# arnavdantuluri/StableTriton

Hardware: AMD Instinct MI355X
Metric: denoise it/s, SDXL UNet 1024x1024 50-step, bs=1 per GPU (higher is better)
Workload: dtype bf16; 1 GPU; SDXL-base UNet, latent 128x128 (1024x1024 px), bs=1/GPU, 50-step Euler-discrete loop, hipGraph mode=step, no CFG; parallelism=prompt-parallel x1, weights=synthetic seed 0, weight_broadcasts=0

## Files before the change

### stabletriton_amd/csrc/dispatch.h

```cpp
#pragma once
#include "gemm_reg.h"
#include "gemm_dma.h"
#include "gemm8p.h"
#ifdef ST_DEV_CONFIGS
#include "../../tools/dev_kernels/gemm4w.h"
void gemm4w_bf16(const GemmArgs& a, hipStream_t st);
void gemm4w_f16(const GemmArgs& a, hipStream_t st);
void gemm4w_fp8(const GemmArgs& a, hipStream_t st);
template <typename T> static inline void gemm4w_call(const GemmArgs& a, hipStream_t st) {
    if constexpr (std::is_same<T, bf16>::value) gemm4w_bf16(a, st);
    else if constexpr (std::is_same<T, f16>::value) gemm4w_f16(a, st);
    else gemm4w_fp8(a, st);
}
#endif

static inline bool colstats_ok(const GemmArgs& a, int bm, bool lnf) {
    const bool ok = a.col_stats && !lnf && (a.N & 3) == 0 && a.rows_per_batch > 0 && a.rows_per_batch % bm == 0 &&
                    cdiv(a.M, bm) <= a.col_tiles_cap;
    if (a.col_rows_out) *a.col_rows_out = ok ? bm : 0;
    return ok;
}

template <typename T, int BM, int BN, int WGM, int WGN, int STAGES, int U, bool CONV, bool GEGLU, bool LNF, bool XA = false>
static void launch_dma_one(const GemmArgs& a, hipStream_t st, int tiles_n) {
    const size_t lds = (size_t)STAGES * U * (BM + BN) * 128 + (size_t)BM * 8 + 1024;
    const int sk = a.splitk > 1 ? a.splitk : 1;
    auto kfn = gemm_dma_kernel<T, BM, BN, WGM, WGN, STAGES, U, CONV, GEGLU, LNF, XA>;
    const bool emit_cols = colstats_ok(a, BM, LNF);
    static unsigned long long lds_ok = 0;
    ensure_dynamic_lds(kfn, lds, &lds_ok);
    GemmArgs b = a;
    {
        static const int force_pm = dev_env_int("ST_GEMM_PANELS", 0);
        const int tiles_m = cdiv(a.M, BM);
        const double abytes = CONV ? (double)a.M * a.Cin * (a.ups ? 0.25 : 1.0) * a.stride * a.stride : (double)a.M * a.K;
        const double wbytes = (double)(GEGLU ? 2 : 1) * a.N * a.K;
        int best_p = 1;
        double best = 1e300;
        for (int pm = 1; pm <= 8; pm *= 2) {
            if (pm > tiles_m) break;
            const double c = abytes * (8.0 / pm) + wbytes * pm;
            if (c < best) { best = c; best_p = pm; }
        }
        if (force_pm > 0) best_p = force_pm > tiles_m ? tiles_m : force_pm;
        b.panel_h = cdiv(tiles_m, best_p);
    }
    const int main_blocks = cdiv(a.M, BM) * tiles_n * sk;
    b.splitk = sk;
    fill_tile_map(b, cdiv(a.M, BM), tiles_n, a.K / ((128 / (int)sizeof(T)) * U));
    static const bool no_helpers = dev_env_int("ST_NO_HELPER_BLOCKS", 0) != 0;
    b.helper_blocks = (b.next_w && main_blocks <= 208 && !no_helpers) ? (256 - main_blocks > 96 ? 96 : 256 - main_blocks) : 0;
    if (!emit_cols) b.col_stats = nullptr;
    fill_next_per(b, main_blocks + b.helper_blocks);
    hipLaunchKernelGGL(kfn, dim3(main_blocks + b.helper_blocks), dim3(WGM * WGN * 64), lds, st, b);
}

template <typename T, int BM, int BN, int WGM, int WGN, int STAGES, int U, bool CONV>
static void launch_dma(const GemmArgs& a, hipStream_t st) {
    if constexpr (!CONV) {
        const bool geglu = a.epi & ST_EPI_GEGLU;
        constexpr bool PAIRS = (BN % 32 == 0);
        if (a.ln_c) {
            if constexpr (PAIRS) {
                if (geglu) { launch_dma_one<T, BM, BN, WGM, WGN, STAGES, U, false, true, true>(a, st, cdiv(a.N, BN / 2)); return; }
            }
            launch_dma_one<T, BM, BN, WGM, WGN, STAGES, U, false, false, true>(a, st, cdiv(a.N, BN));
            return;
        }
        if constexpr (PAIRS) {
            if (geglu) { launch_dma_one<T, BM, BN, WGM, WGN, STAGES, U, false, true, false>(a, st, cdiv(a.N, BN / 2)); return; }
        }
    }
    launch_dma_one<T, BM, BN, WGM, WGN, STAGES, U, CONV, false, false>(a, st, cdiv(a.N, BN));
}

enum { CFG_64x64_S4 = 0, CFG_64x64_S8 = 1, CFG_64x64_S4_U2 = 2, CFG_128x64_S4 = 3, CFG_128x64_S3_U2 = 4,
       CFG_128x128_S3 = 5, CFG_64x64_S3 = 6, CFG_64x64_W8 = 7, CFG_128x64_W8 = 8, CFG_128x128_W8 = 9,
       CFG_64x128_W8 = 10, CFG_64x128_W8_S6 = 11, CFG_128x64_W8_S6 = 12, CFG_128x128_W8_S4 = 13, CFG_64x64_W8_S8 = 14, CFG_64x128_W8_U2 = 15, CFG_128x64_W8_U2 = 16, CFG_64x64_W8_U2 = 17, CFG_256x256_W8 = 18, CFG_256x128_W8 = 19, CFG_128x128_W8_S2 = 20, CFG_128x64_W8_S3 = 21, CFG_64x128_W8_S3 = 22, CFG_128x320_W8 = 23, CFG_128x256_W8 = 24, CFG_64x320_W8 = 25, CFG_64x80_W4 = 26, CFG_128x80_W8 = 27, CFG_128x160_W8 = 28, CFG_128x128_N4_S2 = 29, CFG_128x64_N4_S3 = 30, CFG_64x128_N4_S3 = 31, CFG_256x160_W8_S2 = 32, CFG_COUNT, CFG_256x256_8P = 100, CFG_256x160_8P = 101, CFG_256x256_4W = 102 };

static inline int cfg_bn(int cfg) {
    switch (cfg) {
        case CFG_64x64_S4: case CFG_64x64_S8: case CFG_64x64_S4_U2: case CFG_128x64_S4: case CFG_128x64_S3_U2: case CFG_64x64_S3:
        case CFG_64x64_W8: case CFG_128x64_W8: case CFG_128x64_W8_S6: case CFG_64x64_W8_S8: case CFG_128x64_W8_U2:
        case CFG_64x64_W8_U2: case CFG_128x64_W8_S3: case CFG_128x64_N4_S3: return 64;
        case CFG_256x256_W8: case CFG_128x256_W8: return 256;
        case CFG_128x320_W8: case CFG_64x320_W8: return 320;
        case CFG_64x80_W4: case CFG_128x80_W8: return 80;
        case CFG_128x160_W8: case CFG_256x160_W8_S2: return 160;
        default: return 128;
    }
}

#ifdef ST_DEV_CONFIGS
extern int g_dbg_cfg, g_dbg_fusek;
#endif
static inline int forced_cfg() {
    static int v = dev_env_int("ST_GEMM_FORCE", -1);
#ifdef ST_DEV_CONFIGS
    if (g_dbg_cfg >= 0) return g_dbg_cfg;
#endif
    return v;
}

#ifndef ST_TW_128x128
#define ST_TW_128x128 1.0
#endif
#ifndef ST_TW_64x128
#define ST_TW_64x128 1.0
#endif
#ifndef ST_TW_128x64
#define ST_TW_128x64 1.0
#endif
#ifndef ST_TW_64x64
#define ST_TW_64x64 1.0
#endif
#ifndef ST_TW_128x80
#define ST_TW_128x80 1.0
#endif
#ifndef ST_TW_128x160
#define ST_TW_128x160 1.0
#endif
#ifndef ST_TW_SPLITK
#define ST_TW_SPLITK 1.0
#endif
#ifndef ST_TW_8P
#define ST_TW_8P 1.1
#endif
static inline double model_tweak(int cfg) {
    switch (cfg) {
        case 9: return ST_TW_128x128;
        case 10: return ST_TW_64x128;
        case 8: return ST_TW_128x64;
        case 7: return ST_TW_64x64;
        case 27: return ST_TW_128x80;
        case 28: return ST_TW_128x160;
        default: return 1.0;
    }
}
#ifndef ST_SPLIT_DENSE_TRIP
#define ST_SPLIT_DENSE_TRIP 1.0
#endif
#ifndef ST_SPLIT_160_TRIP
#define ST_SPLIT_160_TRIP 0.8
#endif
template <typename T, bool CONV>
static int gemm_dispatch(const GemmArgs& a_in, hipStream_t st, int depth = 0) {
    GemmArgs a = a_in;
    if (a.Ng == 0) a.Ng = a.N;
    const long n_eff = (a.epi & ST_EPI_GEGLU) ? 2L * a.N : a.N;
    auto tiles = [&](int bm, int bn) { return (long)cdiv(a.M, bm) * cdiv(n_eff, bn); };
    constexpr int KB = 128 / (int)sizeof(T);
    const char* who = CONV ? "conv2d" : "linear";
    if constexpr (frag2<T>()) {
        if (a.K % KB != 0) return st_fail("%s: fp8 / split fp32 operands need K to be a multiple of %d", who, KB);
    } else if (a.K % KB != 0) {
        if (a.stats_chunks_out) *a.stats_chunks_out = 0;
        if (tiles(128, 128) >= 240) launch_cfg<T, 128, 128, 2, 2, CONV>(a, st);
        else if (tiles(128, 64) >= 200) launch_cfg<T, 128, 64, 2, 2, CONV>(a, st);
        else launch_cfg<T, 64, 64, 2, 2, CONV>(a, st);
        return st_check_launch(who);
    }
    if constexpr (std::is_same<T, float>::value) {
        GemmArgs b = a;
        b.stats_chunks = cdiv(a.N, 64);
        if (a.stats_chunks_out) *a.stats_chunks_out = a.row_stats ? b.stats_chunks : 0;
        launch_dma<T, 64, 64, 2, 2, 4, 1, CONV>(b, st);
        return st_check_launch(who);
    } else {
        const bool even2 = (a.K % (2 * KB) == 0);
        struct Cand { int cfg, bm, bn; double trip_us; };
        static const Cand cands[] = {{CFG_128x128_W8, 128, 128, 0.53}, {CFG_64x128_W8, 64, 128, 0.34}, {CFG_128x64_W8, 128, 64, 0.32},
                                     {CFG_64x64_W8, 64, 64, 0.19}, {CFG_128x320_W8, 128, 320, 1.9}, {CFG_64x320_W8, 64, 320, 1.1},
                                     {CFG_256x128_W8, 256, 128, 0.72}, {CFG_128x80_W8, 128, 80, 0.37}, {CFG_128x160_W8, 128, 160, 0.66}};
        static const int sks[] = {1, 2, 3, 4, 6, 8};
        static const int force_sk = dev_env_int("ST_GEMM_SPLITK", -1);
        const int nk = a.K / KB;
        const long ncols = (a.epi & ST_EPI_GEGLU) ? 2L * a.N : a.N;
        const bool can_split = a.partial && !a.ln_c && force_sk != 0 && force_sk != 1;
        int cfg = CFG_64x64_W8, sk = 1;
        double best = 1e30;
        auto small_model = [&](long ncols_, int* cfg_out, int* sk_out) {
            auto tiles_ = [&](int bm, int bn) { return (long)cdiv(a.M, bm) * cdiv(ncols_, bn); };
            double best_ = 1e30;
            for (const Cand& c : cands) {
                if (frag2<T>() && c.bn == 320) continue;
                if (is_split<T>() && c.cfg == CFG_256x128_W8) continue;
                if ((a.epi & ST_EPI_GEGLU) && c.bn % 32 != 0) continue;
                const long nt = tiles_(c.bm, c.bn);
                const double trip = (is_split<T>() && c.cfg == CFG_128x160_W8 ? ST_SPLIT_160_TRIP : c.trip_us * (is_split<T>() && !CONV ? ST_SPLIT_DENSE_TRIP : 1.0)) * (CONV ? 1.6 : 1.0) * ((!CONV && sizeof(T) == 2) ? model_tweak(c.cfg) : 1.0);
                for (int k_ : sks) {
                    if (k_ > 1 && (!can_split || nk / k_ < 4 || nt > 16384)) break;
                    const double slab_mb = (double)k_ * nt * c.bm * c.bn * 4.0 / 1e6;
                    if (k_ > 1 && slab_mb * 1e6 + 65536 > (double)a.partial_bytes) break;
                    const double rounds = (double)((nt * k_ + 255) / 256);
                    const double in_round = (double)(nt * k_ < 256 ? nt * k_ : 256);
                    const double trip_bw = in_round * (c.bm + c.bn) * 128.0 / 14.0e6;
                    const double cost = rounds * (cdiv(nk, k_) * (trip > trip_bw ? trip : trip_bw) + 3.0) * (rounds > 1.0 ? 1.3 : 1.0) + (k_ > 1 ? (2.1 + 0.4 * slab_mb) * ((!CONV && sizeof(T) == 2) ? ST_TW_SPLITK : 1.0) : 0.0);
                    if (cost < best_) { best_ = cost; if (cfg_out) *cfg_out = c.cfg; if (sk_out) *sk_out = k_; }
                }
            }
            return best_;
        };
        best = small_model(ncols, &cfg, &sk);
        if constexpr (!CONV && sizeof(T) <= 2) {
            const int f = forced_cfg();
            double c256 = 1e30, c160 = 1e30;
            if (gemm8p_applies(a, 256, KB)) c256 = (double)((tiles(256, 256) + 255) / 256) * (nk * 1.65 + 4.0);
            if (gemm8p_applies(a, 160, KB)) c160 = (double)((tiles(256, 160) + 255) / 256) * (nk * 1.52 + 4.0);
#ifdef ST_DEV_CONFIGS
            if (f == CFG_256x256_4W && gemm4w_applies(a, KB)) { gemm4w_call<T>(a, st); return st_check_launch(who); }
#endif
            static const bool no_colsplit = dev_env_int("ST_NO_COLSPLIT", 0) != 0;
            if (f < 0 && depth == 0 && !no_colsplit && c256 < 1e29 && !a.row_stats && !a.col_stats && !a.q8_out && !a.sp_out && !a.row_scale) {
                const long tm = a.M / 256, total = tiles(256, 256);
                const long rem = total % 256;
                if (total > 256 && rem > 0 && rem <= 128 && 256 % tm == 0) {
                    const long full_cols = (total / 256) * (256 / tm);
                    const long rem_rows = n_eff - full_cols * 256;
                    const double c_full = (double)(total / 256) * (nk * 1.65 + 4.0);
                    const double c_split = c_full + small_model(rem_rows, nullptr, nullptr) + 2.5;
                    const double c_whole = c256 < c160 ? c256 : c160;
                    if (c_split < 0.93 * (c_whole < best ? c_whole : best)) {
                        const int bno = (a.epi & ST_EPI_GEGLU) ? 128 : 256;
                        const long n1 = full_cols * bno;
                        typedef typename OutT<T>::type TO_;
                        GemmArgs a1 = a, a2 = a;
                        a1.N = (int)n1;
                        a1.next_w = (const char*)a.W + (size_t)n1 * a.K * sizeof(T); a1.next_bytes = (size_t)(a.N - n1) * a.K * sizeof(T); a1.next_row_lines = 0; a1.next_lead_shift = 0;
                        a2.N = a.N - (int)n1;
                        a2.W = (const char*)a.W + (size_t)n1 * a.K * sizeof(T);
                        a2.C = (char*)a.C + (size_t)n1 * sizeof(TO_);
                        if (a.bias) a2.bias = (const char*)a.bias + (size_t)n1 * sizeof(TO_);
                        if (a.residual) a2.residual = (const char*)a.residual + (size_t)n1 * sizeof(TO_);
                        if (a.ln_c) { a2.ln_c = a.ln_c + n1; a2.ln_d = a.ln_d + n1; }
                        if (a.col_scale) a2.col_scale = a.col_scale + n1;
                        if (a.stats_chunks_out) *a.stats_chunks_out = 0;
                        gemm8p_launch<T, 256, 2, 4>(a1, st);
                        if (int e = st_check_launch(who)) return e;
                        return gemm_dispatch<T, CONV>(a2, st, depth + 1);
                    }
                }
            }
            const bool take256 = f == CFG_256x256_8P || (f < 0 && c256 <= c160 && c256 < ST_TW_8P * best);
            const bool take160 = f == CFG_256x160_8P || (f < 0 && c160 < c256 && c160 < ST_TW_8P * best);
            if (take256 && c256 < 1e29) { gemm8p_launch<T, 256, 2, 4>(a, st); return st_check_launch(who); }
            if (take160 && c160 < 1e29) { gemm8p_launch<T, 160, 4, 2>(a, st); return st_check_launch(who); }
        }
        if constexpr (!CONV && is_split<T>()) {
            const int f = forced_cfg();
            double c160 = 1e30;
            if (gemm8p_applies(a, 160, KB)) c160 = (double)((tiles(256, 160) + 255) / 256) * (nk * 1.15 + 5.0);
            if (c160 < 1e29 && (f == CFG_256x160_8P || (f < 0 && c160 < 0.9 * best))) { gemm8p_launch<T, 160, 4, 2>(a, st); return st_check_launch(who); }
        }
        GemmArgs b = a;
#ifdef ST_DEV_CONFIGS
        {
            static const int small_cfg = dev_env_int("ST_GEMM_SMALL_CFG", -1);
            if (small_cfg >= 0 && small_cfg < CFG_COUNT && tiles(128, 128) < 150 && sk == 1) cfg = small_cfg;
        }
#endif
        {
            static const int env_fk = dev_env_int("ST_GEMM_FUSEK", -1);
            int force_fk = env_fk;
#ifdef ST_DEV_CONFIGS
            if (g_dbg_cfg >= 0) force_fk = g_dbg_fusek;
#endif
            const int f = forced_cfg();
            if (f >= 0 && f < CFG_COUNT) {
                const bool u2 = (f == CFG_64x64_S4_U2 || f == CFG_128x64_S3_U2 || f == CFG_64x128_W8_U2 || f == CFG_128x64_W8_U2 ||
                                 f == CFG_64x64_W8_U2);
                if (!u2 || even2) { cfg = f; sk = (force_fk > 1 && can_split) ? (force_fk > nk ? nk : force_fk) : 1; }
            }
        }
        if (sk > 1) {
            int bm = 128;
            if (cfg == CFG_64x64_W8 || cfg == CFG_64x128_W8 || cfg == CFG_64x320_W8 || cfg == CFG_64x80_W4) bm = 64;
            if (cfg == CFG_256x128_W8 || cfg == CFG_256x160_W8_S2) bm = 256;
            const long nt = tiles(bm, cfg_bn(cfg));
            if (nt <= 16384 && (size_t)sk * nt * bm * cfg_bn(cfg) * 4 + 65536 <= a.partial_bytes) {
                b.splitk = sk; b.tile_counters = (int*)a.partial; b.partial = a.partial + 16384;
            }
        }
        b.stats_chunks = cdiv(a.N, cfg_bn(cfg));
        if (a.row_stats && b.stats_chunks > a.stats_capacity) return st_fail("%s: row_stats buffer holds %d chunks, %d needed", who, a.stats_capacity, b.stats_chunks);
        if (a.stats_chunks_out) *a.stats_chunks_out = a.row_stats ? b.stats_chunks : 0;
        switch (cfg) {
            case CFG_64x64_W8: launch_dma<T, 64, 64, 4, 2, 4, 1, CONV>(b, st); break;
            case CFG_128x64_W8: launch_dma<T, 128, 64, 4, 2, 4, 1, CONV>(b, st); break;
            case CFG_64x128_W8: launch_dma<T, 64, 128, 2, 4, 4, 1, CONV>(b, st); break;
            case CFG_256x128_W8: launch_dma<T, 256, 128, 4, 2, 3, 1, CONV>(b, st); break;
            case CFG_128x320_W8: launch_dma<T, 128, 320, 4, 2, 2, 1, CONV>(b, st); break;
            case CFG_64x320_W8: launch_dma<T, 64, 320, 2, 4, 3, 1, CONV>(b, st); break;
            case CFG_128x80_W8: launch_dma<T, 128, 80, 8, 1, 4, 1, CONV>(b, st); break;
            case CFG_128x160_W8:
                if constexpr (is_split<T>()) launch_dma<T, 128, 160, 4, 2, 4, 1, CONV>(b, st);
                else launch_dma<T, 128, 160, 8, 1, 4, 1, CONV>(b, st);
                break;
#ifdef ST_DEV_CONFIGS
            case CFG_64x80_W4: launch_dma<T, 64, 80, 4, 1, 6, 1, CONV>(b, st); break;
            case CFG_128x256_W8: launch_dma<T, 128, 256, 4, 2, 3, 1, CONV>(b, st); break;
            case CFG_64x64_S4: launch_dma<T, 64, 64, 2, 2, 4, 1, CONV>(b, st); break;
            case CFG_64x64_S8: launch_dma<T, 64, 64, 2, 2, 8, 1, CONV>(b, st); break;
            case CFG_64x64_S4_U2: launch_dma<T, 64, 64, 2, 2, 4, 2, CONV>(b, st); break;
            case CFG_128x64_S4: launch_dma<T, 128, 64, 2, 2, 4, 1, CONV>(b, st); break;
            case CFG_128x64_S3_U2: launch_dma<T, 128, 64, 2, 2, 3, 2, CONV>(b, st); break;
            case CFG_128x128_S3: launch_dma<T, 128, 128, 2, 2, 3, 1, CONV>(b, st); break;
            case CFG_64x64_S3: launch_dma<T, 64, 64, 2, 2, 3, 1, CONV>(b, st); break;
            case CFG_128x128_N4_S2: launch_dma<T, 128, 128, 2, 2, 2, 1, CONV>(b, st); break;
            case CFG_128x64_N4_S3: launch_dma<T, 128, 64, 2, 2, 3, 1, CONV>(b, st); break;
            case CFG_64x128_N4_S3: launch_dma<T, 64, 128, 2, 2, 3, 1, CONV>(b, st); break;
            case CFG_256x160_W8_S2: launch_dma<T, 256, 160, 4, 2, 2, 1, CONV>(b, st); break;
            case CFG_64x128_W8_S6: launch_dma<T, 64, 128, 2, 4, 6, 1, CONV>(b, st); break;
            case CFG_128x64_W8_S6: launch_dma<T, 128, 64, 4, 2, 6, 1, CONV>(b, st); break;
            case CFG_128x128_W8_S4: launch_dma<T, 128, 128, 2, 4, 3, 1, CONV>(b, st); break;
            case CFG_64x64_W8_S8: launch_dma<T, 64, 64, 4, 2, 8, 1, CONV>(b, st); break;
            case CFG_64x128_W8_U2: launch_dma<T, 64, 128, 2, 4, 3, 2, CONV>(b, st); break;
            case CFG_128x64_W8_U2: launch_dma<T, 128, 64, 4, 2, 3, 2, CONV>(b, st); break;
            case CFG_64x64_W8_U2: launch_dma<T, 64, 64, 4, 2, 4, 2, CONV>(b, st); break;
            case CFG_256x256_W8: launch_dma<T, 256, 256, 2, 4, 2, 1, CONV>(b, st); break;
            case CFG_128x128_W8_S2: launch_dma<T, 128, 128, 2, 4, 2, 1, CONV>(b, st); break;
            case CFG_128x64_W8_S3: launch_dma<T, 128, 64, 4, 2, 3, 1, CONV>(b, st); break;
            case CFG_64x128_W8_S3: launch_dma<T, 64, 128, 2, 4, 3, 1, CONV>(b, st); break;
#endif
            default: launch_dma<T, 128, 128, 2, 4, 4, 1, CONV>(b, st); break;
        }
        return st_check_launch(who);
    }
}


static inline void take_hint(GemmArgs& a, const void* next_w, size_t next_bytes) {
    const size_t row_lines = (next_bytes >> 40) & 0xfffff, shift = (next_bytes >> 60) & 3;
    next_bytes &= ((size_t)1 << 40) - 1;
    a.next_row_lines = 0; a.next_lead_shift = 0;
    if (next_w && row_lines && (row_lines >> shift) >= 2 && next_bytes >= (row_lines << 7)) {
        const size_t rows = (next_bytes >> 7) / row_lines;
        a.next_row_lines = (unsigned)row_lines; a.next_lead_shift = (unsigned)shift;
        next_bytes = (rows << shift) << 7;
    }
    a.next_w = next_bytes ? next_w : nullptr;
    a.next_bytes = next_w ? next_bytes : 0;
}

static inline int check_epilogue(const char* who, const GemmArgs& a) {
    ST_REQUIRE(!(a.epi & ST_EPI_BIAS) || a.bias, "%s: ST_EPI_BIAS without bias pointer", who);
    ST_REQUIRE(!(a.epi & ST_EPI_RESIDUAL) || a.residual, "%s: ST_EPI_RESIDUAL without residual pointer", who);
    ST_REQUIRE(!(a.epi & ST_EPI_ROWBIAS) || (a.rowbias && a.rows_per_batch > 0), "%s: ST_EPI_ROWBIAS needs rowbias and rows_per_batch", who);
    ST_REQUIRE(!((a.epi & ST_EPI_GEGLU) && (a.epi & ST_EPI_SILU)), "%s: GEGLU and SILU are exclusive", who);
    return 0;
}
```

### stabletriton_amd/csrc/gemm8p.h

```cpp
#pragma once
#include "gemm_dma.h"

template <int BN, int WGM, int WGN> constexpr bool TILE_OK_SPLIT() { return (256 / WGM / 16) * (BN / WGN / 16) <= 20; }
template <typename T, bool GEGLU, bool LNF, int BN = 256, int WGM = 2, int WGN = 4, bool DIRECT = false>
__global__ __launch_bounds__(512) void gemm8p_kernel(const GemmArgs p) {
    static_assert(sizeof(T) <= 2 || is_split<T>(), "16-bit elements (bf16 / f16), e4m3 bytes, or split fp32 operands (strict mode: 256 x 160 tiles)");
    static_assert(!is_split<T>() || (TILE_OK_SPLIT<BN, WGM, WGN>()), "split operands carry two accumulator sets: wave tiles of at most 64 x 80");
    constexpr int BM = 256, NW = 8;
    constexpr int KB = 128 / (int)sizeof(T);
    constexpr int EV = 16 / (int)sizeof(T);
    typedef typename OutT<T>::type TO;
    static_assert(WGM * WGN == NW && BM % (32 * WGM) == 0 && BN % (16 * WGN) == 0 && (!GEGLU || BN % 32 == 0), "wave layout");
    constexpr int WTM = BM / WGM, WTN = BN / WGN, TM = WTM / 16, TN = WTN / 16;
    constexpr int TMH = TM / 2, TN0 = (TN + 1) / 2, TN1 = TN - TN0;
    constexpr int RA = WGM * TMH * 16, RB0 = WGN * TN0 * 16, RB1 = WGN * TN1 * 16;
    static_assert(RA == 128 && RB0 <= 128 && RB1 <= 128 && RB0 % 8 == 0 && RB1 % 8 == 0, "a region is at most sixteen 8-row pieces");
    constexpr int HA = RA * 128, HB0 = RB0 * 128, HB1 = RB1 * 128;
    constexpr int TILE_B = 2 * HA + HB0 + HB1;
    constexpr int BNO = GEGLU ? BN / 2 : BN;
    typedef typename Mma<T>::Frag Frag;
    typedef typename std::conditional<frag2<T>(), u32x4, Frag>::type Half;
    extern __shared__ __attribute__((aligned(16))) char lds[];
    char* const lnrows = lds + 2 * TILE_B;
    char* const dump = lnrows + BM * 8;

    const int t = threadIdx.x, lane = t & 63;
    const int wave = __builtin_amdgcn_readfirstlane(t >> 6);
    const int wm = wave / WGN, wn = wave - wm * WGN;
    const int tiles_m = p.M / BM;
    const int nblk = gridDim.x - p.helper_blocks, bid = blockIdx.x;
    if (bid >= nblk) {
        unsigned int sink = 0;
        touch_next_weights(p, sink, true);
        retire_touches(sink);
        return;
    }
    const TileId tid = tile_of_block(p, bid, nblk);
    const int tile_m = tid.tile_m, tile_n = tid.tile_n;
    const int m0 = tile_m * BM, n0 = tile_n * BNO;
#ifdef ST_PROBE8
    unsigned long long pr_t0 = __builtin_readcyclecounter(), pr_t1 = 0, pr_t2 = 0, pr_r0 = __builtin_amdgcn_s_memrealtime();
#endif
    const T* __restrict__ Ap = (const T*)p.A;
    const T* __restrict__ Wp = (const T*)p.W;
    const T* zeros = reinterpret_cast<const T*>(g_zero16);

    const int lr = lane >> 3;
    const int lc = (lane & 7) ^ lr;
    const T* a_src[2];
    const T* b0_src[2];
    const T* b1_src[2];
    auto w_row = [&](int c) { return GEGLU ? (c < BN / 2 ? (size_t)(n0 + c) : (size_t)p.Ng + n0 + (c - BN / 2)) : (size_t)(n0 + c); };
    auto w_row_direct = [&](int wc, int j, int rho) {
        const DirectCol dc = direct_col<TN, GEGLU>(j, rho);
        return (size_t)(dc.gate ? p.Ng : 0) + n0 + wc * (GEGLU ? WTN / 2 : WTN) + dc.col;
    };
#pragma unroll
    for (int e = 0; e < 2; ++e) {
        const int idx = (2 * wave + e) * 8 + lr;
        a_src[e] = Ap + (size_t)(m0 + (idx / (TMH * 16)) * WTM + (idx % (TMH * 16))) * p.lda + lc * EV;
        const int i0 = idx < RB0 ? idx : 0, i1 = idx < RB1 ? idx : 0;
        if constexpr (DIRECT) {
            const int in0 = i0 % (TN0 * 16), in1 = i1 % (TN1 * 16);
            b0_src[e] = Wp + w_row_direct(i0 / (TN0 * 16), in0 >> 4, in0 & 15) * p.K + lc * EV;
            b1_src[e] = Wp + w_row_direct(i1 / (TN1 * 16), TN0 + (in1 >> 4), in1 & 15) * p.K + lc * EV;
        } else {
            b0_src[e] = Wp + w_row((i0 / (TN0 * 16)) * WTN + (i0 % (TN0 * 16))) * p.K + lc * EV;
            b1_src[e] = Wp + w_row((i1 / (TN1 * 16)) * WTN + TN0 * 16 + (i1 % (TN1 * 16))) * p.K + lc * EV;
        }
    }
    const size_t a_half = (size_t)(TMH * 16) * p.lda;
    const int nk = p.K / KB;

    auto issue_half = [&](int kt, int region) {
#ifdef ST_PROBE8
        if (p.korder & 2) kt = nk;
#endif
        const int roff = region == 0 ? 0 : region == 1 ? HA : region == 2 ? 2 * HA : 2 * HA + HB0;
        const int rrows = region < 2 ? RA : region == 2 ? RB0 : RB1;
        const unsigned dst = lds_addr_of(lds) + (kt & 1) * TILE_B + roff + (2 * wave) * 1024;
#pragma unroll
        for (int e = 0; e < 2; ++e) {
            const bool live = kt < nk && (2 * wave + e) * 8 < rrows;
            const T* src = region < 2 ? a_src[e] + (region & 1) * a_half : region == 2 ? b0_src[e] : b1_src[e];
            src = live ? src + (size_t)kt * KB : zeros;
            dma16_at<0>(src, live ? dst + e * 1024 : lds_addr_of(lds) + 2 * TILE_B + BM * 8);
        }
    };

    unsigned int touch_sink = 0;
    {
        auto touch_at = [&](const char* a) {
            a = (const char*)((uintptr_t)a & ~(uintptr_t)3);
            asm volatile("global_load_dword %0, %1, off" : "+v"(touch_sink) : "v"(a) : "memory");
        };
        auto touch = [&](const void* base, long byte_off, int nbytes) {
            for (int o = t * 128; o < nbytes; o += 512 * 128) touch_at((const char*)base + byte_off + o);
        };
        if (p.epi & ST_EPI_BIAS) {
            touch(p.bias, (long)n0 * (long)sizeof(TO), BNO * (int)sizeof(TO));
            if (GEGLU) touch(p.bias, ((long)p.Ng + n0) * (long)sizeof(TO), BNO * (int)sizeof(TO));
        }
        if (LNF) {
            touch(p.ln_c, (long)n0 * 4, BNO * 4); touch(p.ln_d, (long)n0 * 4, BNO * 4);
            if (GEGLU) { touch(p.ln_c, ((long)p.Ng + n0) * 4, BNO * 4); touch(p.ln_d, ((long)p.Ng + n0) * 4, BNO * 4); }
        }
        if (p.epi & ST_EPI_RESIDUAL) {
            constexpr int lines = (BNO * (int)sizeof(TO) + 127) / 128;
            for (int o = t; o < BM * lines; o += 512) {
                const int r = o / lines, l = o - r * lines;
                touch_at((const char*)p.residual + ((size_t)(m0 + r) * p.ldr + n0) * sizeof(TO) + l * 128);
            }
        }
    }
    LnRowSum<2> ln_sum;
    if constexpr (LNF) {
        const float2* st2 = reinterpret_cast<const float2*>(p.ln_stats);
        const int row = t >> 1, part = t & 1;
        ln_sum.load(st2 + (size_t)(m0 + row) * p.ln_chunks, p.ln_chunks, part);
    }
    issue_half(0, 0); issue_half(0, 2); issue_half(0, 3); issue_half(0, 1); issue_half(1, 0); issue_half(1, 2); issue_half(1, 3);
    if constexpr (LNF) {
        const float2* st2 = reinterpret_cast<const float2*>(p.ln_stats);
        const int row = t >> 1, part = t & 1;
        float a1, a2;
        ln_sum.finish(st2 + (size_t)(m0 + row) * p.ln_chunks, p.ln_chunks, part, a1, a2);
        const float mean = a1 / (float)p.K;
        const float rstd = rsqrtf(fmaxf(a2 / (float)p.K - mean * mean, 0.f) + p.ln_eps);
        if (part == 0) reinterpret_cast<float2*>(lnrows)[row] = make_float2(mean, rstd);
        asm volatile("s_waitcnt lgkmcnt(0)" ::: "memory");
    }
    wait_vmcnt<8>();
    __builtin_amdgcn_s_barrier();
    asm volatile("" ::"v"(touch_sink));
    if (wave >= 4) __builtin_amdgcn_s_barrier();

    f32x4 acc[TM][TN];
    f32x4 corr[is_split<T>() ? TM : 1][is_split<T>() ? TN : 1];
#pragma unroll
    for (int i = 0; i < TM; ++i)
#pragma unroll
        for (int j = 0; j < TN; ++j) {
            acc[i][j] = (f32x4){0.f, 0.f, 0.f, 0.f};
            if constexpr (is_split<T>()) corr[i][j] = (f32x4){0.f, 0.f, 0.f, 0.f};
        }

    const int r16 = lane & 15, q = lane >> 4;
    int a_off[2], b0_off[2], b1_off[2];
#pragma unroll
    for (int kk = 0; kk < 2; ++kk) {
        const int sw = ((4 * kk + q) ^ (r16 & 7)) << 4;
        a_off[kk] = (wm * TMH * 16 + r16) * 128 + sw;
        b0_off[kk] = 2 * HA + (wn * TN0 * 16 + r16) * 128 + sw;
        b1_off[kk] = 2 * HA + HB0 + (wn * TN1 * 16 + r16) * 128 + sw;
    }
    constexpr int NKK = frag2<T>() ? 1 : 2;
    Frag fa[TMH][NKK], fb[TN][NKK];
    auto read_op = [&](const char* base, const int (&off)[2], Frag (&dst)[NKK]) {
        if constexpr (frag2<T>()) {
            const Half lo = *reinterpret_cast<const Half*>(base + off[0]), hi = *reinterpret_cast<const Half*>(base + off[1]);
            dst[0] = Frag{(int)lo[0], (int)lo[1], (int)lo[2], (int)lo[3], (int)hi[0], (int)hi[1], (int)hi[2], (int)hi[3]};
        } else {
#pragma unroll
            for (int kk = 0; kk < 2; ++kk) dst[kk] = *reinterpret_cast<const Frag*>(base + off[kk]);
        }
    };
    auto read_a = [&](const char* tile, int h) {
#pragma unroll
        for (int i = 0; i < TMH; ++i) read_op(tile + h * HA + i * 2048, a_off, fa[i]);
    };
    auto read_b = [&](const char* tile) {
#pragma unroll
        for (int j = 0; j < TN0; ++j) read_op(tile + j * 2048, b0_off, fb[j]);
#pragma unroll
        for (int j = 0; j < TN1; ++j) read_op(tile + j * 2048, b1_off, fb[TN0 + j]);
    };
    auto half_tile = [&](auto mh_) {
        constexpr int mh = decltype(mh_)::value;
#ifdef ST_PROBE8
        if (p.korder & 1) return;
#endif
        __builtin_amdgcn_s_setprio(1);
#pragma unroll
        for (int kk = 0; kk < NKK; ++kk)
#pragma unroll
            for (int i = 0; i < TMH; ++i)
#pragma unroll
                for (int j = 0; j < TN; ++j) {
                    if constexpr (is_split<T>()) Mma<T>::run2(acc[mh * TMH + i][j], corr[mh * TMH + i][j], fb[j][kk], fa[i][kk]);
                    else Mma<T>::run(acc[mh * TMH + i][j], fb[j][kk], fa[i][kk]);
                }
        __builtin_amdgcn_s_setprio(0);
    };
#define ST_PHASE_SYNC()                                   \
    __builtin_amdgcn_sched_barrier(0);                    \
    wait_vmcnt<8>();                                      \
    __builtin_amdgcn_s_barrier();                         \
    __builtin_amdgcn_sched_barrier(0)
#define ST_PHASE_END()                                    \
    __builtin_amdgcn_sched_barrier(0);                    \
    __builtin_amdgcn_s_barrier();                         \
    __builtin_amdgcn_sched_barrier(0)
    typedef std::integral_constant<int, 0> I0;
    typedef std::integral_constant<int, 1> I1;
#ifdef ST_PROBE8
    pr_t1 = __builtin_readcyclecounter();
#endif
    for (int kt = 0; kt < nk; ++kt) {
        const char* tile = lds + (kt & 1) * TILE_B;
        read_a(tile, 0); read_b(tile);
        issue_half(kt + 1, 1);
        ST_PHASE_SYNC();
        half_tile(I0{});
        ST_PHASE_END();
        read_a(tile, 1);
        issue_half(kt + 2, 0); issue_half(kt + 2, 2); issue_half(kt + 2, 3);
        ST_PHASE_SYNC();
        half_tile(I1{});
        ST_PHASE_END();
    }
#undef ST_PHASE_SYNC
#undef ST_PHASE_END
    if (wave < 4) __builtin_amdgcn_s_barrier();
    wait_vmcnt<0>();
    __builtin_amdgcn_s_barrier();
#ifdef ST_PROBE8
    pr_t2 = __builtin_readcyclecounter();
#endif
    if constexpr (is_split<T>()) {
#pragma unroll
        for (int i = 0; i < TM; ++i)
#pragma unroll
            for (int j = 0; j < TN; ++j)
#pragma unroll
                for (int e = 0; e < 4; ++e) acc[i][j][e] = __builtin_fmaf(corr[i][j][e], ST_SPLIT_INV, acc[i][j][e]);
    }
    if constexpr (DIRECT)
        direct_epilogue<TO, TM, TN, WTM, WTN, WGM, WGN, GEGLU, LNF>(p, acc, m0, n0, tile_n, wm, wn, r16, q, lds, reinterpret_cast<const float2*>(lnrows),
                                                                    lds_addr_of(lds) + 2 * TILE_B + BM * 8);
    else
        staged_epilogue<TO, BM, BN, WGM, WGN, TM, TN, GEGLU, 2 * TILE_B, !LNF, is_fp8<T>()>(p, acc, m0, n0, tile_n, wm, r16, q, ColsPlain{wn, WTN}, lds,
                                                                            reinterpret_cast<const float2*>(lnrows));
#ifdef ST_PROBE8
    asm volatile("s_waitcnt vmcnt(0)" ::: "memory");
    if (p.partial && t == 0) {
        unsigned long long* o = reinterpret_cast<unsigned long long*>(reinterpret_cast<char*>(p.partial) + 65536) + (size_t)bid * 8;
        o[0] = pr_t0; o[1] = pr_t1; o[2] = pr_t2; o[3] = __builtin_readcyclecounter(); o[4] = pr_r0; o[5] = __builtin_amdgcn_s_memrealtime();
    }
#endif
}

static inline bool gemm8p_applies(const GemmArgs& a, int bn, int kb = 64) {
    const long n_rows = (a.epi & ST_EPI_GEGLU) ? 2L * a.N : a.N;
    return a.M % 256 == 0 && n_rows % bn == 0 && a.K % kb == 0 && a.K >= 2 * kb && a.N % 8 == 0 &&
           !(a.epi & ST_EPI_ROWBIAS) && (!a.row_stats || !(a.epi & ST_EPI_GEGLU));
}

template <typename T, bool GEGLU, bool LNF, int BN, int WGM, int WGN, bool DIRECT = false>
static void gemm8p_go(const GemmArgs& a, hipStream_t st) {
    constexpr size_t lds = 2 * (size_t)(2 * 128 * 128 + BN * 128) + 256 * 8 + 1024;
    auto kfn = gemm8p_kernel<T, GEGLU, LNF, BN, WGM, WGN, DIRECT>;
    static unsigned long long lds_ok = 0;
    ensure_dynamic_lds(kfn, lds, &lds_ok);
    GemmArgs b = a;
    const int tiles_m = a.M / 256, tiles_n = (int)(((a.epi & ST_EPI_GEGLU) ? 2L * a.N : a.N) / BN);
    {
        const double abytes = (double)a.M * a.K, wbytes = (double)tiles_n * BN * a.K;
        int best_p = 1;
        double best = 1e300;
        for (int pm = 1; pm <= 8 && pm <= tiles_m; pm *= 2) {
            const double c = abytes * (8.0 / pm) + wbytes * pm;
            if (c < best) { best = c; best_p = pm; }
        }
        b.panel_h = cdiv(tiles_m, best_p);
    }
    const int main_blocks = tiles_m * tiles_n;
    b.splitk = 1;
    fill_tile_map(b, tiles_m, tiles_n, 0);
    b.helper_blocks = (b.next_w && main_blocks <= 208) ? (256 - main_blocks > 96 ? 96 : 256 - main_blocks) : 0;
    b.stats_chunks = tiles_n;
    if (a.stats_chunks_out) *a.stats_chunks_out = a.row_stats ? b.stats_chunks : 0;
    if (!colstats_ok(a, 256, LNF)) b.col_stats = nullptr;
    fill_next_per(b, main_blocks + b.helper_blocks);
    hipLaunchKernelGGL(kfn, dim3(main_blocks + b.helper_blocks), dim3(512), lds, st, b);
}

template <typename T>
static inline bool gemm8p_direct(const GemmArgs& a, bool tall) {
    if constexpr (sizeof(T) != 2) return false;
    static const bool off = dev_env_int("ST_8P_STAGED", 0) != 0;
    if (off || direct_flags(a, a.ln_c != nullptr, tall) < 0) return false;
    auto al16 = [](const void* p_) { return ((uintptr_t)p_ & 15) == 0; };
    return a.ldc % 8 == 0 && al16(a.C) && (!(a.epi & ST_EPI_RESIDUAL) || (a.ldr % 8 == 0 && al16(a.residual))) && al16(a.bias) && al16(a.ln_c) && al16(a.ln_d);
}

template <typename T, int BN, int WGM, int WGN>
static void gemm8p_launch(const GemmArgs& a, hipStream_t st) {
    const bool geglu = a.epi & ST_EPI_GEGLU;
    if constexpr (sizeof(T) == 2) {
        if (gemm8p_direct<T>(a, 256 / WGM / 16 >= 8)) {
            if (a.ln_c) { if (geglu) gemm8p_go<T, true, true, BN, WGM, WGN, true>(a, st); else gemm8p_go<T, false, true, BN, WGM, WGN, true>(a, st); }
            else { if (geglu) gemm8p_go<T, true, false, BN, WGM, WGN, true>(a, st); else gemm8p_go<T, false, false, BN, WGM, WGN, true>(a, st); }
            return;
        }
    }
    if (a.ln_c) { if (geglu) gemm8p_go<T, true, true, BN, WGM, WGN>(a, st); else gemm8p_go<T, false, true, BN, WGM, WGN>(a, st); }
    else { if (geglu) gemm8p_go<T, true, false, BN, WGM, WGN>(a, st); else gemm8p_go<T, false, false, BN, WGM, WGN>(a, st); }
}
```

### stabletriton_amd/csrc/gemm_api.hip

```cpp
#include "gemm_core.h"

#ifdef ST_DEV_CONFIGS
int g_dbg_cfg = -1, g_dbg_fusek = -1;
extern "C" void st_debug_force_gemm(int cfg, int fusek) { g_dbg_cfg = cfg; g_dbg_fusek = fusek; }
#endif

static int run_dense(const GemmArgs& a, int dtype, hipStream_t st) {
    switch (dtype) {
        case ST_BF16: return gemm_dense_bf16(a, st);
        case ST_F16: return gemm_dense_f16(a, st);
        case ST_F32S: return gemm_dense_f32s(a, st);
        default: return gemm_dense_f32(a, st);
    }
}

static int check_q8(const char* who, GemmArgs& a, void* q8, long ldq8, const float* q8_inv_scale, unsigned int* q8_amax) {
    if (!q8) return 0;
    ST_REQUIRE(q8_inv_scale && q8_amax, "%s: the e4m3 copy needs its scale and its amax slots", who);
    ST_REQUIRE(a.N % 8 == 0 && ldq8 % 8 == 0 && (uintptr_t)q8 % 8 == 0, "%s: e4m3 copy: N and its row stride must be multiples of 8", who);
    a.q8_out = q8; a.q8_ld = ldq8; a.q8_inv_scale = q8_inv_scale; a.q8_amax = q8_amax;
    return 0;
}

static int linear_impl(const void* x, const void* W, const void* bias, const void* residual, const void* rowbias, void* y,
                       int M, int N, int K, long lda, long ldc, long ldr, int rows_per_batch, int epilogue, int dtype,
                       void* workspace, size_t workspace_bytes, float* row_stats, int row_stats_capacity,
                       int* row_stats_chunks, float* col_stats, int col_stats_tiles, int* col_stats_rows,
                       void* q8, long ldq8, const float* q8_inv_scale, unsigned int* q8_amax,
                       const void* next_weights, size_t next_weights_bytes, void* stream) {
    if (col_stats_rows) *col_stats_rows = 0;
    ST_REQUIRE(x && W && y, "linear: null pointer");
    ST_REQUIRE(M > 0 && N > 0 && K > 0, "linear: bad shape M=%d N=%d K=%d", M, N, K);
    ST_REQUIRE(st_dtype_ok_gemm(dtype), "linear: unsupported dtype %d", dtype);
    const int vec = st_dtype_is16(dtype) ? 8 : (dtype == ST_F32S ? 32 : 4);
    ST_REQUIRE(K % vec == 0 && lda % vec == 0, "linear: K=%d and lda=%ld must be multiples of %d", K, lda, vec);
    ST_REQUIRE(ldc % 4 == 0 && (!(epilogue & ST_EPI_RESIDUAL) || ldr % 4 == 0), "linear: ldc/ldr must be multiples of 4");
    ST_REQUIRE(((uintptr_t)x | (uintptr_t)W) % 16 == 0 && (uintptr_t)y % 16 == 0, "linear: pointers must be 16-byte aligned");
    GemmArgs a = {};
    a.A = x; a.W = W; a.bias = bias; a.residual = residual; a.rowbias = rowbias; a.C = y;
    a.M = M; a.N = N; a.K = K; a.lda = lda; a.ldc = ldc; a.ldr = ldr; a.rows_per_batch = rows_per_batch; a.epi = epilogue;
    a.splitk = 1; a.partial = (float*)workspace; a.partial_bytes = workspace ? workspace_bytes : 0;
    ST_REQUIRE(!row_stats || !(epilogue & ST_EPI_GEGLU), "linear: row_stats with GEGLU is not supported");
    a.row_stats = row_stats; a.stats_capacity = row_stats_capacity; a.stats_chunks_out = row_stats_chunks;
    a.col_stats = col_stats; a.col_tiles_cap = col_stats_tiles; a.col_rows_out = col_stats_rows;
    take_hint(a, next_weights, next_weights_bytes);
#ifdef ST_PROBE8
    { const char* e_ = getenv("ST_PROBE_KNOB"); a.korder = e_ ? atoi(e_) : 0; }
#endif
    if (int e = check_epilogue("linear", a)) return e;
    if (q8) {
        ST_REQUIRE(st_dtype_is16(dtype), "linear: the e4m3 copy is emitted by the 16-bit kernels");
        if (int e = check_q8("linear", a, q8, ldq8, q8_inv_scale, q8_amax)) return e;
    }
    if (int e = st_take_split_arm("linear", M, N, !st_dtype_is16(dtype) && N % 32 == 0, &a.sp_out)) return e;
    return run_dense(a, dtype, (hipStream_t)stream);
}

extern "C" int st_linear(const void* x, const void* W, const void* bias, const void* residual, const void* rowbias, void* y,
                         int M, int N, int K, long lda, long ldc, long ldr, int rows_per_batch, int epilogue, int dtype,
                         void* workspace, size_t workspace_bytes, float* row_stats, int row_stats_capacity,
                         int* row_stats_chunks, float* col_stats, int col_stats_tiles, int* col_stats_rows,
                         const void* next_weights, size_t next_weights_bytes, void* stream) {
    return linear_impl(x, W, bias, residual, rowbias, y, M, N, K, lda, ldc, ldr, rows_per_batch, epilogue, dtype, workspace, workspace_bytes,
                       row_stats, row_stats_capacity, row_stats_chunks, col_stats, col_stats_tiles, col_stats_rows, nullptr, 0, nullptr, nullptr,
                       next_weights, next_weights_bytes, stream);
}

extern "C" int st_linear_emit8(const void* x, const void* W, const void* bias, const void* residual, const void* rowbias, void* y,
                               int M, int N, int K, long lda, long ldc, long ldr, int rows_per_batch, int epilogue, int dtype,
                               void* workspace, size_t workspace_bytes, float* row_stats, int row_stats_capacity,
                               int* row_stats_chunks, float* col_stats, int col_stats_tiles, int* col_stats_rows,
                               void* q8, long ldq8, const float* q8_inv_scale, unsigned int* q8_amax,
                               const void* next_weights, size_t next_weights_bytes, void* stream) {
    ST_REQUIRE(q8, "linear_emit8: null e4m3 output");
    return linear_impl(x, W, bias, residual, rowbias, y, M, N, K, lda, ldc, ldr, rows_per_batch, epilogue, dtype, workspace, workspace_bytes,
                       row_stats, row_stats_capacity, row_stats_chunks, col_stats, col_stats_tiles, col_stats_rows, q8, ldq8, q8_inv_scale, q8_amax,
                       next_weights, next_weights_bytes, stream);
}

extern "C" int st_ln_linear(const void* x, const float* row_stats, int row_stats_chunks, const void* Wg, const float* c,
                            const float* d, void* y, int M, int N, int K, long lda, long ldc, float eps, int epilogue,
                            int dtype, const void* next_weights, size_t next_weights_bytes, void* stream) {
    ST_REQUIRE(x && Wg && c && d && y && row_stats, "ln_linear: null pointer");
    ST_REQUIRE(row_stats_chunks > 0, "ln_linear: the producer emitted no row statistics");
    ST_REQUIRE(M > 0 && N > 0 && K > 0, "ln_linear: bad shape M=%d N=%d K=%d", M, N, K);
    ST_REQUIRE(st_dtype_ok_gemm(dtype), "ln_linear: unsupported dtype %d", dtype);
    const int kb = st_dtype_is16(dtype) ? 64 : 32;
    ST_REQUIRE(K % kb == 0 && lda % (dtype == ST_F32S ? 32 : kb / 8) == 0, "ln_linear: K=%d must be a multiple of %d", K, kb);
// ... 159 lines not shown
```

Baseline: 77.50 it/s.

## Add software-pipelined main loop to 256x160 8-wave GEMM kernel

Adds a PIPE variant of the 256x160 bf16/f16 direct-store 8-wave GEMM kernel that double-buffers operand fragments in registers. It splits each K step into two half-segments and interleaves LDS reads and DMA issues between MFMA instructions using sched_group_barrier. This replaces the ping-pong wave-group barrier scheme with per-segment barriers, meant to hide LDS read latency and overlap loads with matrix math. It also adds a dry-run dispatch hook that reports the chosen GEMM config for debugging, and restricts the 160-wide path to operands whose offsets fit in 32 bits, at the cost of higher register pressure.

```diff
diff --git a/stabletriton_amd/csrc/dispatch.h b/stabletriton_amd/csrc/dispatch.h
--- a/stabletriton_amd/csrc/dispatch.h
+++ b/stabletriton_amd/csrc/dispatch.h
@@ -94,6 +94,7 @@
 #ifdef ST_DEV_CONFIGS
 extern int g_dbg_cfg, g_dbg_fusek;
 #endif
+extern int g_last_gemm_cfg, g_gemm_dry;
 static inline int forced_cfg() {
     static int v = dev_env_int("ST_GEMM_FORCE", -1);
 #ifdef ST_DEV_CONFIGS
@@ -155,6 +156,8 @@
         if (a.K % KB != 0) return st_fail("%s: fp8 / split fp32 operands need K to be a multiple of %d", who, KB);
     } else if (a.K % KB != 0) {
         if (a.stats_chunks_out) *a.stats_chunks_out = 0;
+        g_last_gemm_cfg = -1;
+        if (g_gemm_dry) return 0;
         if (tiles(128, 128) >= 240) launch_cfg<T, 128, 128, 2, 2, CONV>(a, st);
         else if (tiles(128, 64) >= 200) launch_cfg<T, 128, 64, 2, 2, CONV>(a, st);
         else launch_cfg<T, 64, 64, 2, 2, CONV>(a, st);
@@ -164,6 +167,8 @@
         GemmArgs b = a;
         b.stats_chunks = cdiv(a.N, 64);
         if (a.stats_chunks_out) *a.stats_chunks_out = a.row_stats ? b.stats_chunks : 0;
+        g_last_gemm_cfg = CFG_64x64_S4;
+        if (g_gemm_dry) return 0;
         launch_dma<T, 64, 64, 2, 2, 4, 1, CONV>(b, st);
         return st_check_launch(who);
     } else {
@@ -208,7 +213,7 @@
             if (gemm8p_applies(a, 256, KB)) c256 = (double)((tiles(256, 256) + 255) / 256) * (nk * 1.65 + 4.0);
             if (gemm8p_applies(a, 160, KB)) c160 = (double)((tiles(256, 160) + 255) / 256) * (nk * 1.52 + 4.0);
 #ifdef ST_DEV_CONFIGS
-            if (f == CFG_256x256_4W && gemm4w_applies(a, KB)) { gemm4w_call<T>(a, st); return st_check_launch(who); }
+            if (f == CFG_256x256_4W && gemm4w_applies(a, KB)) { g_last_gemm_cfg = CFG_256x256_4W; if (g_gemm_dry) return 0; gemm4w_call<T>(a, st); return st_check_launch(who); }
 #endif
             static const bool no_colsplit = dev_env_int("ST_NO_COLSPLIT", 0) != 0;
             if (f < 0 && depth == 0 && !no_colsplit && c256 < 1e29 && !a.row_stats && !a.col_stats && !a.q8_out && !a.sp_out && !a.row_scale) {
@@ -235,22 +240,26 @@
                         if (a.ln_c) { a2.ln_c = a.ln_c + n1; a2.ln_d = a.ln_d + n1; }
                         if (a.col_scale) a2.col_scale = a.col_scale + n1;
                         if (a.stats_chunks_out) *a.stats_chunks_out = 0;
-                        gemm8p_launch<T, 256, 2, 4>(a1, st);
-                        if (int e = st_check_launch(who)) return e;
-                        return gemm_dispatch<T, CONV>(a2, st, depth + 1);
+                        if (!g_gemm_dry) {
+                            gemm8p_launch<T, 256, 2, 4>(a1, st);
+                            if (int e = st_check_launch(who)) return e;
+                        }
+                        const int e2 = gemm_dispatch<T, CONV>(a2, st, depth + 1);
+                        g_last_gemm_cfg += 1000;
+                        return e2;
                     }
                 }
             }
             const bool take256 = f == CFG_256x256_8P || (f < 0 && c256 <= c160 && c256 < ST_TW_8P * best);
             const bool take160 = f == CFG_256x160_8P || (f < 0 && c160 < c256 && c160 < ST_TW_8P * best);
-            if (take256 && c256 < 1e29) { gemm8p_launch<T, 256, 2, 4>(a, st); return st_check_launch(who); }
-            if (take160 && c160 < 1e29) { gemm8p_launch<T, 160, 4, 2>(a, st); return st_check_launch(who); }
+            if (take256 && c256 < 1e29) { g_last_gemm_cfg = CFG_256x256_8P; if (g_gemm_dry) return 0; gemm8p_launch<T, 256, 2, 4>(a, st); return st_check_launch(who); }
+            if (take160 && c160 < 1e29) { g_last_gemm_cfg = CFG_256x160_8P; if (g_gemm_dry) return 0; gemm8p_launch<T, 160, 4, 2>(a, st); return st_check_launch(who); }
         }
         if constexpr (!CONV && is_split<T>()) {
             const int f = forced_cfg();
             double c160 = 1e30;
             if (gemm8p_applies(a, 160, KB)) c160 = (double)((tiles(256, 160) + 255) / 256) * (nk * 1.15 + 5.0);
-            if (c160 < 1e29 && (f == CFG_256x160_8P || (f < 0 && c160 < 0.9 * best))) { gemm8p_launch<T, 160, 4, 2>(a, st); return st_check_launch(who); }
+            if (c160 < 1e29 && (f == CFG_256x160_8P || (f < 0 && c160 < 0.9 * best))) { g_last_gemm_cfg = CFG_256x160_8P; if (g_gemm_dry) return 0; gemm8p_launch<T, 160, 4, 2>(a, st); return st_check_launch(who); }
         }
         GemmArgs b = a;
 #ifdef ST_DEV_CONFIGS
@@ -284,6 +293,8 @@
         b.stats_chunks = cdiv(a.N, cfg_bn(cfg));
         if (a.row_stats && b.stats_chunks > a.stats_capacity) return st_fail("%s: row_stats buffer holds %d chunks, %d needed", who, a.stats_capacity, b.stats_chunks);
         if (a.stats_chunks_out) *a.stats_chunks_out = a.row_stats ? b.stats_chunks : 0;
+        g_last_gemm_cfg = cfg;
+        if (g_gemm_dry) return 0;
         switch (cfg) {
             case CFG_64x64_W8: launch_dma<T, 64, 64, 4, 2, 4, 1, CONV>(b, st); break;
             case CFG_128x64_W8: launch_dma<T, 128, 64, 4, 2, 4, 1, CONV>(b, st); break;
@@ -322,7 +333,7 @@
             case CFG_128x64_W8_S3: launch_dma<T, 128, 64, 4, 2, 3, 1, CONV>(b, st); break;
             case CFG_64x128_W8_S3: launch_dma<T, 64, 128, 2, 4, 3, 1, CONV>(b, st); break;
 #endif
-            default: launch_dma<T, 128, 128, 2, 4, 4, 1, CONV>(b, st); break;
+            default: g_last_gemm_cfg = CFG_128x128_W8; launch_dma<T, 128, 128, 2, 4, 4, 1, CONV>(b, st); break;
         }
         return st_check_launch(who);
     }
diff --git a/stabletriton_amd/csrc/gemm8p.h b/stabletriton_amd/csrc/gemm8p.h
--- a/stabletriton_amd/csrc/gemm8p.h
+++ b/stabletriton_amd/csrc/gemm8p.h
@@ -2,10 +2,14 @@
 #include "gemm_dma.h"
 
 template <int BN, int WGM, int WGN> constexpr bool TILE_OK_SPLIT() { return (256 / WGM / 16) * (BN / WGN / 16) <= 20; }
-template <typename T, bool GEGLU, bool LNF, int BN = 256, int WGM = 2, int WGN = 4, bool DIRECT = false>
+template <typename T, int BN, bool GEGLU, bool LNF, bool DIRECT> constexpr bool gemm8p_pipe() {
+    return BN == 160 && sizeof(T) == 2 && DIRECT && (GEGLU || !LNF);
+}
+template <typename T, bool GEGLU, bool LNF, int BN = 256, int WGM = 2, int WGN = 4, bool DIRECT = false, bool PIPE = gemm8p_pipe<T, BN, GEGLU, LNF, DIRECT>()>
 __global__ __launch_bounds__(512) void gemm8p_kernel(const GemmArgs p) {
     static_assert(sizeof(T) <= 2 || is_split<T>(), "16-bit elements (bf16 / f16), e4m3 bytes, or split fp32 operands (strict mode: 256 x 160 tiles)");
     static_assert(!is_split<T>() || (TILE_OK_SPLIT<BN, WGM, WGN>()), "split operands carry two accumulator sets: wave tiles of at most 64 x 80");
+    static_assert(!PIPE || (BN == 160 && sizeof(T) == 2), "the pipelined loop: 256 x 160 tiles of 16-bit operands");
     constexpr int BM = 256, NW = 8;
     constexpr int KB = 128 / (int)sizeof(T);
     constexpr int EV = 16 / (int)sizeof(T);
@@ -120,6 +124,7 @@
         ln_sum.load(st2 + (size_t)(m0 + row) * p.ln_chunks, p.ln_chunks, part);
     }
     issue_half(0, 0); issue_half(0, 2); issue_half(0, 3); issue_half(0, 1); issue_half(1, 0); issue_half(1, 2); issue_half(1, 3);
+    if constexpr (PIPE) issue_half(1, 1);
     if constexpr (LNF) {
         const float2* st2 = reinterpret_cast<const float2*>(p.ln_stats);
         const int row = t >> 1, part = t & 1;
@@ -133,7 +138,9 @@
     wait_vmcnt<8>();
     __builtin_amdgcn_s_barrier();
     asm volatile("" ::"v"(touch_sink));
-    if (wave >= 4) __builtin_amdgcn_s_barrier();
+    if constexpr (!PIPE) {
+        if (wave >= 4) __builtin_amdgcn_s_barrier();
+    }
 
     f32x4 acc[TM][TN];
     f32x4 corr[is_split<T>() ? TM : 1][is_split<T>() ? TN : 1];
@@ -201,11 +208,124 @@
     __builtin_amdgcn_sched_barrier(0);                    \
     __builtin_amdgcn_s_barrier();                         \
     __builtin_amdgcn_sched_barrier(0)
+#define ST_SEGMENT_END()                                  \
+    __builtin_amdgcn_sched_barrier(0);                    \
+    wait_vmcnt<8>();                                      \
+    asm volatile("s_waitcnt lgkmcnt(0)" ::: "memory");    \
+    __builtin_amdgcn_s_barrier();                         \
+    __builtin_amdgcn_sched_barrier(0)
     typedef std::integral_constant<int, 0> I0;
     typedef std::integral_constant<int, 1> I1;
 #ifdef ST_PROBE8
     pr_t1 = __builtin_readcyclecounter();
 #endif
+    if constexpr (PIPE) {
+        Frag pa[2][TMH][NKK], pb[2][TN][NKK];
+        static_assert((TMH * 16) % 8 == 0, "a piece of eight rows lies inside one wave's half");
+        const T* a_ub[2];
+        unsigned b_vo[2][2];
+        const T* const w_ub = Wp + (size_t)n0 * p.K;
+        const unsigned a_vo = (unsigned)((lr * p.lda + lc * EV) * (long)sizeof(T));
+#pragma unroll
+        for (int e = 0; e < 2; ++e) {
+            const int idx0 = (2 * wave + e) * 8;
+            a_ub[e] = Ap + (size_t)(m0 + (idx0 / (TMH * 16)) * WTM + (idx0 % (TMH * 16))) * p.lda;
+            b_vo[0][e] = (unsigned)((const char*)b0_src[e] - (const char*)w_ub);
+            b_vo[1][e] = (unsigned)((const char*)b1_src[e] - (const char*)w_ub);
+        }
+        auto issue_pipe = [&](int kt, auto region_, auto par_) {
+            constexpr int region = decltype(region_)::value, PAR = decltype(par_)::value;
+#ifdef ST_PROBE8
+            if (p.korder & 2) kt = nk;
+#endif
+            constexpr int roff = region == 0 ? 0 : region == 1 ? HA : region == 2 ? 2 * HA : 2 * HA + HB0;
+            constexpr int rrows = region < 2 ? RA : region == 2 ? RB0 : RB1;
+            const unsigned dst = lds_addr_of(lds) + PAR * TILE_B + roff + (2 * wave) * 1024;
+#pragma unroll
+            for (int e = 0; e < 2; ++e) {
+                const bool live = kt < nk && (2 * wave + e) * 8 < rrows;
+                const T* ub = region < 2 ? a_ub[e] + (region & 1) * a_half : w_ub;
+                const unsigned vo = region < 2 ? a_vo : b_vo[region - 2][e];
+                const char* src = (live ? (const char*)(ub + (size_t)kt * KB) : (const char*)zeros) + (size_t)(live ? vo : 0u);
+                dma16_at<0>(src, live ? dst + e * 1024 : lds_addr_of(lds) + 2 * TILE_B + BM * 8);
+            }
+        };
+        typedef std::integral_constant<int, 2> I2;
+        typedef std::integral_constant<int, 3> I3;
+        auto seg = [&](int kt, auto h_, auto par_, auto mm_) {
+            constexpr int h = decltype(h_)::value, PAR = decltype(par_)::value;
+            constexpr bool MM = decltype(mm_)::value;
+            const char* cur = lds + PAR * TILE_B;
+            const char* nxt = lds + (PAR ^ 1) * TILE_B;
+            if constexpr (h == 0) {
+#pragma unroll
+                for (int i = 0; i < TMH; ++i) read_op(cur + HA + i * 2048, a_off, pa[1][i]);
+                issue_pipe(kt + 2, I0{}, par_); issue_pipe(kt + 2, I2{}, par_); issue_pipe(kt + 2, I3{}, par_);
+            } else {
+#pragma unroll
+                for (int i = 0; i < TMH; ++i) read_op(nxt + i * 2048, a_off, pa[0][i]);
+#pragma unroll
+                for (int j = 0; j < TN0; ++j) read_op(nxt + j * 2048, b0_off, pb[PAR ^ 1][j]);
+#pragma unroll
+                for (int j = 0; j < TN1; ++j) read_op(nxt + j * 2048, b1_off, pb[PAR ^ 1][TN0 + j]);
+                issue_pipe(kt + 2, I1{}, par_);
+            }
+            if constexpr (MM) {
+#pragma unroll
+                for (int kk = 0; kk < NKK; ++kk)
+#pragma unroll
+                    for (int i = 0; i < TMH; ++i)
+#pragma unroll
+                        for (int j = 0; j < TN; ++j) Mma<T>::run(acc[h * TMH + i][j], pb[PAR][j][kk], pa[h][i][kk]);
+                constexpr int n_rd = (h == 0 ? TMH : TMH + TN) * NKK, n_dma = h == 0 ? 6 : 2, n_mm = TMH * TN * NKK;
+                static_assert(n_rd + n_dma < n_mm, "a gap per read and per DMA");
+#pragma unroll
+                for (int r = 0; r < n_rd; ++r) {
+                    __builtin_amdgcn_sched_group_barrier(0x008, 1, 0);
+                    __builtin_amdgcn_sched_group_barrier(0x100, 1, 0);
+                }
+#pragma unroll
+                for (int e = 0; e < n_dma; ++e) {
+                    __builtin_amdgcn_sched_group_barrier(0x008, 1, 0);
+                    __builtin_amdgcn_sched_group_barrier(0x020, 1, 0);
+                }
+                __builtin_amdgcn_sched_group_barrier(0x008, n_mm - n_rd - n_dma, 0);
+            }
+#ifdef ST_PROBE8
+            if constexpr (!MM) {
+#pragma unroll
+                for (int kk = 0; kk < NKK; ++kk) {
+#pragma unroll
+                    for (int i = 0; i < TMH; ++i) asm volatile("" ::"v"(pa[h ^ 1][i][kk]));
+#pragma unroll
+                    for (int j = 0; j < TN; ++j) asm volatile("" ::"v"(pb[PAR ^ 1][j][kk]));
+                }
+            }
+#endif
+            ST_SEGMENT_END();
+        };
+        auto run = [&](auto mm_) {
+            for (int kt = 0; kt < nk; kt += 2) {
+                seg(kt, I0{}, I0{}, mm_);
+                seg(kt, I1{}, I0{}, mm_);
+                if (kt + 1 >= nk) break;
+                seg(kt + 1, I0{}, I1{}, mm_);
+                seg(kt + 1, I1{}, I1{}, mm_);
+            }
+        };
+#pragma unroll
+        for (int i = 0; i < TMH; ++i) read_op(lds + i * 2048, a_off, pa[0][i]);
+#pragma unroll
+        for (int j = 0; j < TN0; ++j) read_op(lds + j * 2048, b0_off, pb[0][j]);
+#pragma unroll
+        for (int j = 0; j < TN1; ++j) read_op(lds + j * 2048, b1_off, pb[0][TN0 + j]);
+        ST_SEGMENT_END();
+#ifdef ST_PROBE8
+        if (p.korder & 1) run(std::false_type{});
+        else
+#endif
+        run(std::true_type{});
+    } else {
     for (int kt = 0; kt < nk; ++kt) {
         const char* tile = lds + (kt & 1) * TILE_B;
         read_a(tile, 0); read_b(tile);
@@ -221,7 +341,9 @@
     }
 #undef ST_PHASE_SYNC
 #undef ST_PHASE_END
+#undef ST_SEGMENT_END
     if (wave < 4) __builtin_amdgcn_s_barrier();
+    }
     wait_vmcnt<0>();
     __builtin_amdgcn_s_barrier();
 #ifdef ST_PROBE8
@@ -253,13 +375,14 @@
 static inline bool gemm8p_applies(const GemmArgs& a, int bn, int kb = 64) {
     const long n_rows = (a.epi & ST_EPI_GEGLU) ? 2L * a.N : a.N;
     return a.M % 256 == 0 && n_rows % bn == 0 && a.K % kb == 0 && a.K >= 2 * kb && a.N % 8 == 0 &&
-           !(a.epi & ST_EPI_ROWBIAS) && (!a.row_stats || !(a.epi & ST_EPI_GEGLU));
-}
-
-template <typename T, bool GEGLU, bool LNF, int BN, int WGM, int WGN, bool DIRECT = false>
-static void gemm8p_go(const GemmArgs& a, hipStream_t st) {
+           !(a.epi & ST_EPI_ROWBIAS) && (!a.row_stats || !(a.epi & ST_EPI_GEGLU)) &&
+           (bn != 160 || (n_rows + a.Ng) * (a.K / kb) * 128L < (1L << 32));
+}
+
+template <typename T, bool GEGLU, bool LNF, int BN, int WGM, int WGN, bool DIRECT, bool PIPE>
+static void gemm8p_run(const GemmArgs& a, hipStream_t st) {
     constexpr size_t lds = 2 * (size_t)(2 * 128 * 128 + BN * 128) + 256 * 8 + 1024;
-    auto kfn = gemm8p_kernel<T, GEGLU, LNF, BN, WGM, WGN, DIRECT>;
+    auto kfn = gemm8p_kernel<T, GEGLU, LNF, BN, WGM, WGN, DIRECT, PIPE>;
     static unsigned long long lds_ok = 0;
     ensure_dynamic_lds(kfn, lds, &lds_ok);
     GemmArgs b = a;
@@ -285,6 +408,16 @@
     hipLaunchKernelGGL(kfn, dim3(main_blocks + b.helper_blocks), dim3(512), lds, st, b);
 }
 
+template <typename T, bool GEGLU, bool LNF, int BN, int WGM, int WGN, bool DIRECT = false>
+static void gemm8p_go(const GemmArgs& a, hipStream_t st) {
+#ifdef ST_DEV_CONFIGS
+    if constexpr (gemm8p_pipe<T, BN, GEGLU, LNF, DIRECT>()) {
+        if (dev_env_int("ST_8P_PINGPONG", 0) != 0) { gemm8p_run<T, GEGLU, LNF, BN, WGM, WGN, DIRECT, false>(a, st); return; }
+    }
+#endif
+    gemm8p_run<T, GEGLU, LNF, BN, WGM, WGN, DIRECT, gemm8p_pipe<T, BN, GEGLU, LNF, DIRECT>()>(a, st);
+}
+
 template <typename T>
 static inline bool gemm8p_direct(const GemmArgs& a, bool tall) {
     if constexpr (sizeof(T) != 2) return false;
diff --git a/stabletriton_amd/csrc/gemm_api.hip b/stabletriton_amd/csrc/gemm_api.hip
--- a/stabletriton_amd/csrc/gemm_api.hip
+++ b/stabletriton_amd/csrc/gemm_api.hip
@@ -4,6 +4,24 @@
 int g_dbg_cfg = -1, g_dbg_fusek = -1;
 extern "C" void st_debug_force_gemm(int cfg, int fusek) { g_dbg_cfg = cfg; g_dbg_fusek = fusek; }
 #endif
+
+int g_last_gemm_cfg = -2, g_gemm_dry = 0;
+extern "C" int st_debug_last_gemm_config(void) { return g_last_gemm_cfg; }
+static int run_dense(const GemmArgs& a, int dtype, hipStream_t st);
+extern "C" int st_debug_gemm_choice(int M, int N, int K, int epilogue, int dtype, int ln_folded, size_t workspace_bytes) {
+    static float dummy[4];
+    GemmArgs a = {};
+    a.A = a.W = a.C = dummy; a.M = M; a.N = N; a.K = K; a.lda = K; a.ldc = N; a.epi = epilogue; a.splitk = 1;
+    if (epilogue & ST_EPI_BIAS) a.bias = dummy;
+    if (epilogue & ST_EPI_RESIDUAL) { a.residual = dummy; a.ldr = N; }
+    if (ln_folded) { a.ln_stats = dummy; a.ln_chunks = 1; a.ln_c = a.ln_d = dummy; a.ln_eps = 1e-5f; }
+    if (workspace_bytes) { a.partial = dummy; a.partial_bytes = workspace_bytes; }
+    g_gemm_dry = 1;
+    g_last_gemm_cfg = -2;
+    const int e = st_dtype_ok_gemm(dtype) ? run_dense(a, dtype, nullptr) : 1;
+    g_gemm_dry = 0;
+    return e ? -2 : g_last_gemm_cfg;
+}
 
 static int run_dense(const GemmArgs& a, int dtype, hipStream_t st) {
     switch (dtype) {
```

New measurement: 77.89 it/s, median of 6. About the same (+0.5%).
